# chanzuckerberg/saber

Measured on AMD Instinct MI355X. Metric: EM slices/sec (1024^2, Hiera-L), higher is better.
Workload: dtype bf16; 1 GPU; 1024x1024 uint16 EM slice -> prep.prepare -> SAM2 AMG (Hiera-L, cfgAMG defaults: npoints=32, crop_n_layers=2 -> 21 crops, 3072 grid prompts + 9216 m2m refinements, multimask) -> dedup/sort -> uint16 label plane; BASELINE configs[1]; weights=seeded synthetic Hiera-L (no checkpoint offline), slices_per_rank=22, engine_handles_per_gpu=2, parallelism=single GPU

## Files before the change

include/saber_amd_kernels.h:

```cpp
#ifndef SABER_AMD_KERNELS_H
#define SABER_AMD_KERNELS_H
#include <stdint.h>
#ifdef __cplusplus
extern "C" {
#endif

const char* saber_k_last_error(void);
int saber_k_init(int device_id);

int saber_k_gemm(const uint16_t* A, const uint16_t* W, const float* bias, const float* res, float* out_f32, uint16_t* out_bf16,
                 int M, int N, int K, int act, int act_last, int pool4, int res_shift, int res_mod, void* stream);

int saber_k_gemm_ld(const uint16_t* A, int lda, const uint16_t* W, int ldw, int w_kpad, const float* bias, const float* res, float* out_f32,
                    uint16_t* out_bf16, int M, int N, int K, int act, void* stream);

int saber_k_gemm_rowln(const uint16_t* A, int lda, const uint16_t* W, int ldw, const float* bias, const float* res, float* out_f32,
                       uint16_t* out_bf16, const float* ln_gamma, const float* ln_beta, float ln_eps, uint16_t* ln_out, int M, int N, int K,
                       void* stream);

int saber_k_mlp_rowln(const uint16_t* A, int lda, const uint16_t* W1, int ldw1, const float* b1, const uint16_t* W2, int ldw2, const float* b2,
                      const float* res, float* out_f32, uint16_t* out_bf16, const float* ln_gamma, const float* ln_beta, float ln_eps,
                      uint16_t* ln_out, int M, int C, void* stream);

int saber_k_layernorm(const float* x, const float* gamma, const float* beta, float eps, float* out_f32, uint16_t* out_bf16,
                      int rows, int C, int act, void* stream);

int saber_k_hiera_attention(const uint16_t* qkv, uint16_t* out, int n_windows, int nk, int heads, int q_pool, void* stream);
int saber_k_hiera_attention_ex(const uint16_t* qkv, uint16_t* out, int n_windows, int nk, int heads, int head_dim, int q_pool,
                               const uint8_t* key_mask, void* stream);

int saber_k_dec_attention(const float* q, const float* k, const float* v, uint16_t* out, int B, int nq, int nk, int heads, int hd,
                          int k_shared, void* stream);

int saber_k_prepare(const void* img, int dtype, int H, int W, float* out, float* ws_dev, uint32_t* minmax_dev, void* stream);

int saber_k_mask_post(const float* lowres, int n, int crop_x0, int crop_y0, int crop_w, int crop_h, int H, int W, float thr,
                      float offset, uint32_t* bits, int32_t* stats, void* stream);
// ... 82 lines not shown
```

saber_amd/_lib.py:

```python
import ctypes as C
import os
import subprocess

_HERE = os.path.dirname(os.path.abspath(__file__))
LIB_PATH = os.path.join(_HERE, "libsaber_amd.so")
CSRC = os.path.join(_HERE, "csrc")


class SaberAmdError(RuntimeError):
    pass


class SaberRangeError(SaberAmdError):
    """SABER_ERR_RANGE: the engine's overflow sentinel found NaN / inf in the 16-bit arithmetic (include/saber_amd.h:
    saber_engine_check_finite) - with fp16 operands, an activation beyond 65 504.  The call's results are invalid."""


SABER_OK, SABER_ERR_INVALID, SABER_ERR_STATE, SABER_ERR_HIP, SABER_ERR_CAPACITY, SABER_ERR_RANGE = 0, -1, -2, -3, -4, -5


def build(verbose: bool = False) -> str:
    r = subprocess.run(["make", "-C", CSRC, "-j8"], capture_output=True, text=True)
    if r.returncode != 0:
        raise SaberAmdError("building libsaber_amd.so failed:\n" + r.stdout[-4000:] + r.stderr[-4000:])
# ... 72 lines not shown
    "saber_classifier_set_weight": (_i, [_vp, C.c_char_p, _vp, _i64p, _i]),
    "saber_classifier_finalize": (_i, [_vp]),
    "saber_classifier_predict": (_i, [_vp, _vp, _i, _i, _vp, _i, _i, _vp, _vp]),
    "saber_classifier_head": (_i, [_vp, _vp, _i, _vp, _vp]),
    "saber_classifier_get_crops": (_i, [_vp, _i, _vp, _vp, _vp]),
    "saber_profile_begin": (_i, [_vp]),
    "saber_profile_end": (_i, [_vp, C.POINTER(ProfileClass), _i]),
    "saber_encoder_flops": (C.c_double, [_vp]),
    "saber_decoder_flops_per_prompt": (C.c_double, []),
    "saber_k_last_error": (C.c_char_p, []),
    "saber_k_init": (_i, [_i]),
    "saber_k_gemm": (_i, [_vp, _vp, _vp, _vp, _vp, _vp, _i, _i, _i, _i, _i, _i, _i, _i, _vp]),
    "saber_k_gemm_ld": (_i, [_vp, _i, _vp, _i, _i, _vp, _vp, _vp, _vp, _i, _i, _i, _i, _vp]),
    "saber_k_gemm_rowln": (_i, [_vp, _i, _vp, _i, _vp, _vp, _vp, _vp, _vp, _vp, _f, _vp, _i, _i, _i, _vp]),
    "saber_k_mlp_rowln": (_i, [_vp, _i, _vp, _i, _vp, _vp, _i, _vp, _vp, _vp, _vp, _vp, _vp, _f, _vp, _i, _i, _vp]),
    "saber_k_layernorm": (_i, [_vp, _vp, _vp, _f, _vp, _vp, _i, _i, _i, _vp]),
    "saber_k_hiera_attention": (_i, [_vp, _vp, _i, _i, _i, _i, _vp]),
    "saber_k_hiera_attention_ex": (_i, [_vp, _vp, _i, _i, _i, _i, _i, _vp, _vp]),
    "saber_k_dec_attention": (_i, [_vp, _vp, _vp, _vp, _i, _i, _i, _i, _i, _i, _vp]),
    "saber_k_prepare": (_i, [_vp, _i, _i, _i, _vp, _vp, _vp, _vp]),
    "saber_k_mask_post": (_i, [_vp, _i, _i, _i, _i, _i, _i, _i, _f, _f, _vp, _vp, _vp]),
    "saber_k_perm_index": (_i, [_i, _i, _i]),
    "saber_k_set_operand_type": (_i, [_i]),
    "saber_k_stream_create_cu_range": (_i, [_i, _i, C.POINTER(_vp)]),
    "saber_k_stream_destroy": (_i, [_vp]),
    "saber_k_host_f32_to_f16": (None, [_vp, _vp, C.c_int64]),
    "saber_k_dec_i2t": (_i, [_vp, C.c_int64, _vp, _vp, _vp, _f, _vp, _vp, _vp, _vp, _vp, _f, _vp, _i, _vp]),
    "saber_k_dec_i2t16": (_i, [_vp, C.c_int64, _vp, _vp, _vp, _f, _vp, _vp, _vp, _vp, _vp, _f, _vp, _i, _i, _vp]),
    "saber_k_dec_t2i": (_i, [_vp, C.c_int64, _vp, _vp, _vp, _f, _vp, _vp, _i, _i, _vp, _vp, _vp, _vp]),
    "saber_k_dec_upscale": (_i, [_vp, _vp, _vp, _vp, _vp, _vp, _vp, _vp, _vp, _i, _i, _vp, _vp, _i, _vp, _vp, _i, _vp, _vp]),
# ... 65 lines not shown
```

saber_amd/csrc/capi_kernels.hip:

```cpp
#include <cmath>
#include <cstring>
#include <string>
#include <vector>

#include "../../include/saber_amd_kernels.h"
#include "common.h"
#include "kernels.h"
#include "engine.h"
#include "exact.h"

#include <atomic>

static thread_local std::string g_kerr;
static int kfail(const char* m) { g_kerr = m ? m : "unknown"; return -1; }
static int kcheck(const char* m) {
    if (m) return kfail(m);
    hipError_t st = hipGetLastError();
    if (st != hipSuccess) return kfail(hipGetErrorString(st));
    return 0;
}

extern "C" const char* saber_k_last_error(void) { return g_kerr.c_str(); }

extern "C" int saber_k_init(int device_id) {
    if (hipSetDevice(device_id) != hipSuccess) return kfail("hipSetDevice failed");
    const char* m = gemm_init_device();
    if (!m) m = gemm_rowln_init_device();
    if (!m) m = gemm_mlp_rowln_init_device();
    if (!m) m = hiera_attention_init_device();
    if (!m) m = image_ops_init_device();
    if (!m) m = decoder_fused_init_device();
    if (!m) m = decoder_t16_init_device();
    if (!m) m = amg_device_init();
    (void)hipGetLastError();
    if (m) return kfail(m);
    return 0;
}

extern "C" int saber_k_gemm(const uint16_t* A, const uint16_t* W, const float* bias, const float* res, float* out_f32,
                            uint16_t* out_bf16, int M, int N, int K, int act, int act_last, int pool4, int res_shift, int res_mod,
                            void* stream) {
    GemmParams p;
    p.A = A; p.lda = K; p.W = W; p.ldw = K; p.bias = bias; p.res = res; p.ldres = N; p.Cf = out_f32; p.ldcf = N; p.Cb = out_bf16; p.ldcb = N;
// ... 44 lines not shown
                                 int M, int C, void* stream) {
    if (!gemm_mlp_rowln_width(C)) return kfail("mlp_rowln: width not built (C must be 144)");
    static thread_local bf16_t* scratch = nullptr;
    static thread_local size_t scratch_elems = 0;
    const size_t need = gemm_mlp_rowln_packed_elems(C);
    if (need > scratch_elems) {
        if (scratch) { (void)hipDeviceSynchronize(); (void)hipFree(scratch); scratch = nullptr; scratch_elems = 0; }
        if (hipMalloc(reinterpret_cast<void**>(&scratch), need * sizeof(bf16_t)) != hipSuccess) return kfail("mlp_rowln: scratch allocation failed");
        scratch_elems = need;
    }
    if (const char* m = launch_pack_mlp_chunks(W1, ldw1, W2, ldw2, C, scratch, (hipStream_t)stream)) return kfail(m);
    GemmParams p;
    p.A = A; p.lda = lda; p.bias1 = b1; p.bias = b2; p.res = res; p.ldres = C; p.Cf = out_f32; p.ldcf = C; p.Cb = out_bf16; p.ldcb = C;
    p.M = M; p.N = C; p.K = C; p.ln_gamma = ln_gamma; p.ln_beta = ln_beta; p.ln_eps = ln_eps; p.ln_out = ln_out; p.ldln = C; p.Wpk = scratch;
    return kcheck(launch_gemm_mlp_rowln(p, (hipStream_t)stream));
}

extern "C" int saber_k_layernorm(const float* x, const float* gamma, const float* beta, float eps, float* out_f32, uint16_t* out_bf16,
                                 int rows, int C, int act, void* stream) {
    LayerNormParams p;
    p.x = x; p.ldx = C; p.gamma = gamma; p.beta = beta; p.eps = eps; p.out_f = out_f32; p.out_bf = out_bf16; p.ldo = C; p.rows = rows; p.C = C; p.act = act;
    return kcheck(launch_layernorm(p, (hipStream_t)stream));
}

extern "C" int saber_k_hiera_attention(const uint16_t* qkv, uint16_t* out, int n_windows, int nk, int heads, int q_pool, void* stream) {
    return kcheck(launch_hiera_attention(qkv, out, n_windows, nk, heads, 72, q_pool, nullptr, (hipStream_t)stream));
}

extern "C" int saber_k_hiera_attention_ex(const uint16_t* qkv, uint16_t* out, int n_windows, int nk, int heads, int head_dim, int q_pool,
                                          const uint8_t* key_mask, void* stream) {
// ... 273 lines not shown
```

saber_amd/csrc/engine.h:

```cpp
#pragma once
#include <hip/hip_runtime.h>
#include <functional>
#include <map>
#include <set>
#include <string>
#include <vector>

#include "../../include/saber_amd.h"
#include "kernels.h"

struct BlockSpec { int din, dout, heads, window, q_stride; };

struct HostTensor { std::vector<int64_t> shape; std::vector<float> data; };

struct LinW { const bf16_t* w = nullptr; const float* b = nullptr; int out = 0, in = 0, ldw = 0; const bf16_t* wpk = nullptr; int wpk_n = 0; const float* wf = nullptr;
              const uint8_t* w8 = nullptr; const uint8_t* sw8 = nullptr; int kp8 = 0, sw_rows = 0; };
struct LnW { const float* g = nullptr; const float* b = nullptr; };

struct BlockW { LnW n1, n2; LinW qkv, proj, fc1, fc2, sc; const bf16_t* mlp_pk = nullptr; };

struct AttnW { LinW q, k, v, o; const bf16_t* pe_proj = nullptr; const bf16_t* img_wT = nullptr; };
struct DecLayerW { AttnW self_attn, t2i, i2t; LnW n1, n2, n3, n4; LinW mlp1, mlp2; };

enum { PC_GEMM = 0, PC_HIERA_ATTN, PC_LAYERNORM, PC_DEC_ATTN, PC_ELEMENTWISE, PC_IMAGE, PC_MASK_POST, PC_DEC_T2I, PC_DEC_I2T, PC_DEC_UPSCALE, PC_GEMM_MX, PC_N };
struct ProfRec { int cls; double flops; double bytes; hipEvent_t a, b; };

struct saber_engine {
    int device = 0;
    std::string trunk;
    int max_images = 1, max_prompts = 64;
    std::string err;
    bool finalized = false;
    int weight_format = 0;
    int precision = 0;
// ... 173 lines not shown
```

saber_amd/csrc/engine.hip:

```cpp
#include "engine.h"

#include <algorithm>
#include <cmath>
#include <cstring>
#include <functional>
#include <utility>

#include "common.h"

static thread_local std::string g_create_err;

int eng_fail(saber_engine* e, int code, const std::string& msg) {
    if (e) e->err = msg; else g_create_err = msg;
    return code;
}

int eng_alloc_bytes(saber_engine* e, void** p, size_t bytes) {
    *p = nullptr;
    if (bytes == 0) bytes = 16;
    hipError_t st = hipMalloc(p, bytes);
    if (st != hipSuccess) return eng_fail(e, SABER_ERR_HIP, std::string("hipMalloc(") + std::to_string(bytes) + "): " + hipGetErrorString(st));
    e->allocs.push_back(*p);
    return SABER_OK;
}
// ... 162 lines not shown
    int ndev = 0;
    if (hipGetDeviceCount(&ndev) != hipSuccess || ndev <= 0) return eng_fail(nullptr, SABER_ERR_HIP, "no HIP device visible: the MI355X engine cannot run");
    if (device_id < 0 || device_id >= ndev) return eng_fail(nullptr, SABER_ERR_INVALID, "device_id out of range");
    if (hipSetDevice(device_id) != hipSuccess) return eng_fail(nullptr, SABER_ERR_HIP, "hipSetDevice failed");
    saber_engine* e = new saber_engine();
    e->device = device_id;
    e->trunk = t;
    e->max_images = max_images;
    e->max_prompts = max_prompts;
    if (const char* g = getenv("SABER_AMD_GRAPHS")) e->graphs_on = atoi(g) != 0;
    if (const char* m = hiera_spec(e, *spec)) { delete e; return eng_fail(nullptr, SABER_ERR_INVALID, m); }
    {
        const char* m = gemm_init_device();
            if (!m) m = gemm_rowln_init_device();
            if (!m) m = gemm_mlp_rowln_init_device();
        if (!m) m = amg_device_init();
        if (!m) m = hiera_attention_init_device();
        if (!m) m = image_ops_init_device();
        if (!m) m = decoder_fused_init_device();
        if (!m) m = decoder_tokens_init_device();
        if (!m) m = decoder_t16_init_device();
        (void)hipGetLastError();
        if (m) { delete e; return eng_fail(nullptr, SABER_ERR_HIP, std::string("kernel attribute setup: ") + m); }
    }
    *out = e;
    return SABER_OK;
}

extern "C" void saber_engine_destroy(saber_engine* e) {
    if (!e) return;
// ... 316 lines not shown
            }
        }
        if (!e->padded && (bs.dout == 144 || bs.dout == 288 || bs.dout == 576)) {
            for (LinW* l : {&w.proj, &w.fc2}) {
                bf16_t* d = nullptr;
                TRY(eng_alloc(e, &d, gemm_rowln_packed_elems(l->out, l->in)));
                if (const char* m = launch_pack_w_kstep(l->w, l->ldw, l->out, l->in, d, nullptr)) return eng_fail(e, SABER_ERR_INVALID, m);
                l->wpk = d;
            }
        }
        if (!e->padded && gemm_mlp_rowln_width(bs.dout) && i + 1 < e->blocks.size() && w.fc1.w && w.fc2.w && !w.fc1.w8 && !w.fc2.w8) {
            bf16_t* d = nullptr;
            TRY(eng_alloc(e, &d, gemm_mlp_rowln_packed_elems(bs.dout)));
            if (const char* m = launch_pack_mlp_chunks(w.fc1.w, w.fc1.ldw, w.fc2.w, w.fc2.ldw, bs.dout, d, nullptr)) return eng_fail(e, SABER_ERR_INVALID, m);
            w.mlp_pk = d;
        }
    }
    {
        const std::string nk = "image_encoder.neck.convs.";
        const int dims[4] = {C0 * 8, C0 * 4, C0 * 2, C0};
        const HostTensor *nw[4], *nb[4];
        for (int i = 0; i < 4; ++i) {
            nw[i] = F.get(nk + std::to_string(i) + ".conv.weight", {256, dims[i], 1, 1});
            nb[i] = F.get(nk + std::to_string(i) + ".conv.bias", {256});
        }
        const HostTensor* nm = F.get("no_mem_embed", {1, 1, 256});
        const HostTensor* s0w = F.get("sam_mask_decoder.conv_s0.weight", {32, 256, 1, 1});
        const HostTensor* s0b = F.get("sam_mask_decoder.conv_s0.bias", {32});
        const HostTensor* s1w = F.get("sam_mask_decoder.conv_s1.weight", {64, 256, 1, 1});
        const HostTensor* s1b = F.get("sam_mask_decoder.conv_s1.bias", {64});
// ... 361 lines not shown
    ENG_KP(e, PC_IMAGE, 0.0, 0.0, launch_resize_normalize(img_dev, H, W, channels, e->crops_dev, n, e->pix, 1024, s));
    ENG_KP(e, PC_IMAGE, 0.0, 0.0, launch_patch_embed(e->pix, e->pe_wt, e->pe_bias, e->pos_table, e->xa, n, e->embed_dim, 1024, s));
    if (e->precision == SABER_PRECISION_EXACT) {
        TRY(exact_encode_blocks(e, n, slot0, s));
        for (int i = 0; i < n; ++i) { e->slot_valid[slot0 + i] = 1; e->slot_shared_valid[slot0 + i] = 0; e->slot_embb_valid[slot0 + i] = 0; }
        return SABER_OK;
    }
    float* x = e->xa;
    float* xalt = e->xb;
    int tokens = 65536;
    int stage = 0;
    static const bool no_rowln = getenv("SABER_AMD_NO_ROWLN") != nullptr;
    const bool fuse = !e->padded && !no_rowln;
    static const bool no_mlpfuse = getenv("SABER_AMD_NO_MLPFUSE") != nullptr;
    const bool mlpfuse = fuse && !no_mlpfuse && !(g_saber_debug_flags & 262144);
    const size_t nblocks = e->blocks.size();
    ENG_KP(e, PC_LAYERNORM, 0.0, 0.0, ln_run(x, e->bw[0].n1, 1e-6f, n * tokens, e->blocks[0].din, nullptr, e->xn, ACT_NONE, s, nullptr, nullptr, 0, e->valid[0], tokens));
    const int snake = (g_saber_debug_flags & 512) ? 0 : 1;
    uint8_t* const xn8 = reinterpret_cast<uint8_t*>(e->xn);
    uint8_t* const hid8 = reinterpret_cast<uint8_t*>(e->hid);
    for (size_t i = 0; i < nblocks; ++i) {
        const BlockSpec& bs = e->blocks[i];
        const BlockW& w = e->bw[i];
        const int N = n * tokens;
        float* xres = x;
        int Nq = N;
        if (bs.din != bs.dout) {
            GemmParams g = mk_gemm(e->xn, bs.din, N, w.sc);
            g.Cf = xalt; g.ldcf = bs.dout; g.pool4 = 1;
            ENG_KP(e, PC_GEMM, 2.0 * g.M * (double)g.N * g.K * g.batch, gemm_bytes(g), launch_gemm(g, s));
            xres = xalt;
            Nq = N / 4;
        }
        if (w.qkv.w8) {
            GemmMxParams g = mk_gemm_mx(e, xn8, e->xn8_s, N, w.qkv);
            g.Cb = e->qkv; g.ldcb = 3 * bs.dout;
            ENG_KP(e, PC_GEMM_MX, 2.0 * g.M * (double)g.N * w.qkv.in, (double)g.M * (g.Kp + 2.0 * g.N), launch_gemm_mx(g, s));
        } else {
            GemmParams g = mk_gemm(e->xn, bs.din, N, w.qkv);
            g.Cb = e->qkv; g.ldcb = 3 * bs.dout;
            g.rev = snake;
            ENG_KP(e, PC_GEMM, 2.0 * g.M * (double)g.N * g.K * g.batch, gemm_bytes(g), launch_gemm(g, s));
        }
        const int nk = bs.window > 0 ? bs.window * bs.window : tokens;
        const uint8_t* kmask = (bs.window == 0 && e->valid[stage]) ? e->kmask2 : nullptr;
        ENG_KP(e, PC_HIERA_ATTN, 4.0 * e->head_dim * (double)N * (bs.q_stride > 1 ? nk / 4 : nk) * bs.heads, 0.0,
               launch_hiera_attention(e->qkv, e->att, N / nk, nk, bs.heads, e->head_dim, bs.q_stride > 1, kmask, s));
        {
            GemmParams g = mk_gemm(e->att, bs.dout, Nq, w.proj);
            g.Cf = xres; g.ldcf = bs.dout; g.res = xres; g.ldres = bs.dout;
            g.ln_gamma = w.n2.g; g.ln_beta = w.n2.b; g.ln_eps = 1e-6f; g.ln_out = e->xn; g.ldln = bs.dout;
            g.rev = snake;
            if (w.fc1.w8) {
                g.ln_gamma = nullptr; g.ln_beta = nullptr; g.ln_out = nullptr;
                ENG_KP(e, PC_GEMM, 2.0 * g.M * (double)g.N * g.K * g.batch, gemm_bytes(g), launch_gemm(g, s));
                ENG_KP(e, PC_LAYERNORM, 0.0, 0.0, launch_ln_mx(xres, bs.dout, w.n2.g, w.n2.b, 1e-6f, bs.dout, xn8, mx_kp(bs.dout), mx_kp(bs.dout), e->xn8_s, e->mx_rows, Nq, s));
            } else if (fuse && gemm_rowln_supported(g)) {
                ENG_KP(e, PC_GEMM, 2.0 * g.M * (double)g.N * g.K * g.batch, gemm_bytes(g, true), launch_gemm_rowln(g, s));
            } else {
                ENG_KP(e, PC_GEMM, 2.0 * g.M * (double)g.N * g.K * g.batch, gemm_bytes(g), launch_gemm(g, s));
                ENG_KP(e, PC_LAYERNORM, 0.0, 0.0, ln_run(xres, w.n2, 1e-6f, Nq, bs.dout, nullptr, e->xn, ACT_NONE, s));
            }
        }
        if (bs.din != bs.dout) { std::swap(x, xalt); tokens /= 4; ++stage; }
        const bool has_next = i + 1 < nblocks;
        if (mlpfuse && has_next && w.mlp_pk) {
            GemmParams g = mk_gemm(e->xn, bs.dout, Nq, w.fc2);
            g.K = bs.dout; g.W = nullptr; g.ldw = 0; g.w_kpad = 0; g.Wpk = w.mlp_pk; g.bias1 = w.fc1.b;
            g.Cf = x; g.ldcf = bs.dout; g.res = x; g.ldres = bs.dout;
            g.rev = 0;
            if ((int)i == e->stage_ends[stage]) { g.Cb = e->sb[stage]; g.ldcb = bs.dout; }
            g.ln_gamma = e->bw[i + 1].n1.g; g.ln_beta = e->bw[i + 1].n1.b; g.ln_eps = 1e-6f; g.ln_out = e->xn; g.ldln = bs.dout;
            const double M = g.M, C = bs.dout;
            ENG_KP(e, PC_GEMM, 2.0 * 2.0 * M * C * 4.0 * C, M * C * (2 + 4 + 4 + 2 + (g.Cb ? 2 : 0)) + 2.0 * 8.0 * C * C, launch_gemm_mlp_rowln(g, s));
            continue;
        }
// ... 591 lines not shown
```

saber_amd/csrc/kernels.h:

```cpp
#pragma once
#include <hip/hip_runtime.h>
#include <stdint.h>
#include <stddef.h>

extern int g_saber_debug_flags;
extern unsigned long long* g_saber_stamp_buf;
int saber_cu_count();
extern thread_local int g_saber_op_f16;
inline bool saber_op_is_f16() { return g_saber_op_f16 != 0; }

typedef uint16_t bf16_t;

enum { ACT_NONE = 0, ACT_GELU = 1, ACT_RELU = 2, ACT_SIGMOID = 3 };

struct GemmParams {
    const bf16_t* A = nullptr; int64_t lda = 0; int64_t strideA = 0;
    const bf16_t* W = nullptr; int64_t ldw = 0; int64_t strideW = 0;
    const float* bias = nullptr; int64_t strideBias = 0;
    const float* res = nullptr; int64_t ldres = 0; int64_t strideRes = 0;
    float* Cf = nullptr; int64_t ldcf = 0; int64_t strideCf = 0;
    bf16_t* Cb = nullptr; int64_t ldcb = 0; int64_t strideCb = 0;
    int M = 0, N = 0, K = 0;
    int act = ACT_NONE;
    int act_last = 0;
// ... 114 lines not shown


namespace op_bf16 {
#include "kernels_op.h"
}
namespace op_f16 {
#include "kernels_op.h"
}
#ifndef SABER_OP_NS
#define SABER_OP_FWD(fn)                                                                                                  \
    template <class... A> inline auto fn(A&&... a) {                                                                      \
        return saber_op_is_f16() ? op_f16::fn(static_cast<A&&>(a)...) : op_bf16::fn(static_cast<A&&>(a)...);              \
    }
#define SABER_OP_INIT(fn)                                                                                                 \
    inline const char* fn() { const char* m = op_bf16::fn(); return m ? m : op_f16::fn(); }
SABER_OP_INIT(gemm_init_device) SABER_OP_INIT(gemm_rowln_init_device) SABER_OP_INIT(gemm_mlp_rowln_init_device) SABER_OP_INIT(hiera_attention_init_device)
SABER_OP_INIT(decoder_fused_init_device) SABER_OP_INIT(decoder_tokens_init_device) SABER_OP_INIT(decoder_t16_init_device)
SABER_OP_FWD(launch_gemm) SABER_OP_FWD(gemm_rowln_supported) SABER_OP_FWD(launch_gemm_rowln) SABER_OP_FWD(gemm_rowln_packed_elems) SABER_OP_FWD(launch_pack_w_kstep)
SABER_OP_FWD(gemm_mlp_rowln_width) SABER_OP_FWD(gemm_mlp_rowln_packed_elems) SABER_OP_FWD(launch_pack_mlp_chunks) SABER_OP_FWD(launch_gemm_mlp_rowln)
SABER_OP_FWD(launch_layernorm) SABER_OP_FWD(launch_gather_rows) SABER_OP_FWD(launch_add_to_bf16) SABER_OP_FWD(launch_hiera_attention)
SABER_OP_FWD(launch_prompt_tokens) SABER_OP_FWD(launch_prompt_tokens_multi) SABER_OP_FWD(launch_mask_embed_src) SABER_OP_FWD(launch_mask_hidden) SABER_OP_FWD(launch_embb_tiles)
SABER_OP_FWD(launch_dec_attention) SABER_OP_FWD(launch_mask_pick) SABER_OP_FWD(launch_iou_live_flags) SABER_OP_FWD(launch_mask_select)
SABER_OP_FWD(launch_dec_fold) SABER_OP_FWD(launch_dec_t2i) SABER_OP_FWD(launch_dec_i2t) SABER_OP_FWD(launch_dec_i2t_t2i) SABER_OP_FWD(launch_dec_upscale) SABER_OP_FWD(launch_dec_tokens)
SABER_OP_FWD(launch_prompt_tokens16) SABER_OP_FWD(launch_dec_tokens16) SABER_OP_FWD(launch_dec_i2t16)
SABER_OP_FWD(launch_mask_post) SABER_OP_FWD(launch_gather_masks) SABER_OP_FWD(launch_label_plane) SABER_OP_FWD(launch_pair_intersections) SABER_OP_FWD(launch_unpermute_nchw)
SABER_OP_FWD(launch_rope) SABER_OP_FWD(launch_softmax_rows) SABER_OP_FWD(launch_conv3x3s2) SABER_OP_FWD(launch_unpack_masks) SABER_OP_FWD(launch_paint_nearest)
SABER_OP_FWD(launch_conv3x3s2_t) SABER_OP_FWD(launch_dwconv7_t) SABER_OP_FWD(launch_dwconv7) SABER_OP_FWD(launch_conv4x4s4) SABER_OP_FWD(launch_resize_plane)
SABER_OP_FWD(launch_flash256) SABER_OP_FWD(launch_gauss_mirror) SABER_OP_FWD(launch_axpy) SABER_OP_FWD(launch_bf16_to_f32)
#undef SABER_OP_FWD
#undef SABER_OP_INIT
#endif
```

saber_amd/csrc/kernels_op.h:

```cpp
const char* launch_gemm(const GemmParams& p, hipStream_t stream);
const char* gemm_init_device();
bool gemm_rowln_supported(const GemmParams& p);
const char* launch_gemm_rowln(const GemmParams& p, hipStream_t stream);
const char* gemm_rowln_init_device();
size_t gemm_rowln_packed_elems(int N, int K);
const char* launch_pack_w_kstep(const bf16_t* W, int ldw, int N, int K, bf16_t* out, hipStream_t s);
bool gemm_mlp_rowln_width(int C);
size_t gemm_mlp_rowln_packed_elems(int C);
const char* launch_pack_mlp_chunks(const bf16_t* W1, int ldw1, const bf16_t* W2, int ldw2, int C, bf16_t* out, hipStream_t s);
const char* launch_gemm_mlp_rowln(const GemmParams& p, hipStream_t stream);
const char* gemm_mlp_rowln_init_device();
const char* launch_layernorm(const LayerNormParams& p, hipStream_t s);
const char* launch_gather_rows(const float* in, int64_t in_rows, float* out, int64_t out_rows, const int* idx, int C, int n_images, hipStream_t s);
const char* launch_add_to_bf16(const float* x, const float* y, int ymod, bf16_t* out_bf, float* out_f, int64_t rows, int C,
                               hipStream_t s);
const char* launch_hiera_attention(const bf16_t* qkv, bf16_t* out, int n_windows, int nk, int heads, int hd, int q_pool,
                                   const uint8_t* kmask, hipStream_t s);
const char* hiera_attention_init_device();
const char* launch_prompt_tokens(const float* pts, const int* labels, int P, PromptWeights w, float* tokens, hipStream_t s);
const char* launch_prompt_tokens_multi(const float* pts, const int* labels, int P, int K, PromptWeights w, float* tokens, hipStream_t s);
const char* launch_mask_embed_src(const float* mask_in, int P, const float* image_embed, XMap emb_map, const float* pos, MaskEmbedWeights w,
                                  float* src_f, bf16_t* src_bf, bf16_t* srcpos_bf, float clamp_abs, hipStream_t s, int raw4_q0 = -1);
const char* launch_mask_hidden(const float* mask_in, int P, MaskEmbedWeights w, bf16_t* h2, float clamp_abs, hipStream_t s, int raw4_q0 = -1);
const char* launch_embb_tiles(const float* emb, const float* b3, float* out, hipStream_t s);
const char* launch_dec_attention(const float* q, const float* k, const float* v, bf16_t* out, int B, int nq, int nk, int heads,
                                 int hd, int64_t q_bs, int64_t k_bs, int64_t v_bs, int64_t o_bs, hipStream_t s);
// ... 45 lines not shown
```

Measured before the change: 7.490 slices/s.

## Fuse stage-0 Hiera QKV, windowed attention, projection and LayerNorm into one kernel

Adds a single kernel for stage-0 Hiera blocks (C=144, 2 heads, 8x8 windows). Per 256-row tile it computes the QKV projection, windowed softmax attention and output projection, then applies residual plus LayerNorm, keeping Q in registers and K/V in LDS. Weights are pre-packed into MFMA tile order and double-buffered through LDS. This removes the global round trips for the qkv and attention tensors and two kernel launches per block, at the cost of a narrowly specialised, register- and LDS-heavy kernel with its own packing path.

```diff
diff --git a/include/saber_amd_kernels.h b/include/saber_amd_kernels.h
--- a/include/saber_amd_kernels.h
+++ b/include/saber_amd_kernels.h
@@ -21,6 +21,10 @@
 int saber_k_mlp_rowln(const uint16_t* A, int lda, const uint16_t* W1, int ldw1, const float* b1, const uint16_t* W2, int ldw2, const float* b2,
                       const float* res, float* out_f32, uint16_t* out_bf16, const float* ln_gamma, const float* ln_beta, float ln_eps,
                       uint16_t* ln_out, int M, int C, void* stream);
+
+int saber_k_attn_rowln(const uint16_t* A, int lda, const uint16_t* Wqkv, int ldwqkv, const float* bqkv, const uint16_t* Wp, int ldwp, const float* bp,
+                       const float* res, float* out_f32, uint16_t* out_bf16, const float* ln_gamma, const float* ln_beta, float ln_eps,
+                       uint16_t* ln_out, int M, int C, int heads, void* stream);
 
 int saber_k_layernorm(const float* x, const float* gamma, const float* beta, float eps, float* out_f32, uint16_t* out_bf16,
                       int rows, int C, int act, void* stream);
diff --git a/saber_amd/_lib.py b/saber_amd/_lib.py
--- a/saber_amd/_lib.py
+++ b/saber_amd/_lib.py
@@ -110,6 +110,7 @@
     "saber_k_gemm_ld": (_i, [_vp, _i, _vp, _i, _i, _vp, _vp, _vp, _vp, _i, _i, _i, _i, _vp]),
     "saber_k_gemm_rowln": (_i, [_vp, _i, _vp, _i, _vp, _vp, _vp, _vp, _vp, _vp, _f, _vp, _i, _i, _i, _vp]),
     "saber_k_mlp_rowln": (_i, [_vp, _i, _vp, _i, _vp, _vp, _i, _vp, _vp, _vp, _vp, _vp, _vp, _f, _vp, _i, _i, _vp]),
+    "saber_k_attn_rowln": (_i, [_vp, _i, _vp, _i, _vp, _vp, _i, _vp, _vp, _vp, _vp, _vp, _vp, _f, _vp, _i, _i, _i, _vp]),
     "saber_k_layernorm": (_i, [_vp, _vp, _vp, _f, _vp, _vp, _i, _i, _i, _vp]),
     "saber_k_hiera_attention": (_i, [_vp, _vp, _i, _i, _i, _i, _vp]),
     "saber_k_hiera_attention_ex": (_i, [_vp, _vp, _i, _i, _i, _i, _i, _vp, _vp]),
diff --git a/saber_amd/csrc/attn_rowln.hip b/saber_amd/csrc/attn_rowln.hip
--- /dev/null
+++ b/saber_amd/csrc/attn_rowln.hip
@@ -0,0 +1,327 @@
+#include "common.h"
+#include "kernels.h"
+#include "rowln_epilogue.h"
+
+typedef s16x4 __attribute__((address_space(3))) * lds_s16x4_ptr_a;
+
+template <int C> struct AttnRowLnCfg {
+    static_assert(C == 144, "built for the stage-0 width: 2 heads of 72");
+    static constexpr int R = 256, HD = 72, NK = (C + 31) / 32, NT = C / 16;
+    static constexpr int TPC = 3;
+    static constexpr int QKV_TILES = 36, TILES = QKV_TILES + NT, NCH = TILES / TPC;
+    static constexpr int TILE_B = NK * 1024;
+    static constexpr int UNITS = TPC * TILE_B / 16, NU = (UNITS + 511) / 512;
+    static constexpr int BUF = NU * 512 * 16;
+    static constexpr int VSTRIDE = 224;
+    static constexpr int K_WIN = 4 * 3 * 1024, V_WIN = 64 * VSTRIDE;
+    static constexpr int K_OFF = 0, V_OFF = K_OFF + 4 * K_WIN, W_OFF = V_OFF + 4 * V_WIN, B_OFF = W_OFF + 2 * BUF;
+    static constexpr int SCR_OFF = K_OFF;
+    static constexpr int LDS = B_OFF + QKV_TILES * 16 * 4;
+    static constexpr size_t W_ELEMS = (size_t)TILES * NK * 512;
+    static constexpr size_t PK_ELEMS = W_ELEMS + (size_t)QKV_TILES * 16 * 2;
+    static constexpr float SCALE = 0.11785113019775793f * 1.4426950408889634f;
+    static_assert(8 * RL_SCR <= 4 * K_WIN, "epilogue scratch must fit into the K images");
+    static_assert(TILES % TPC == 0 && (QKV_TILES / 2) % TPC == 0, "chunks must not straddle a head");
+    static_assert(LDS <= 160 * 1024, "LDS budget");
+};
+
+template <int C>
+__global__ __launch_bounds__(512) void gemm_rowln_attn_kernel(GemmParams p) {
+    using CF = AttnRowLnCfg<C>;
+    constexpr int R = CF::R, NK = CF::NK, NT = CF::NT, NCH = CF::NCH, NU = CF::NU, VS = CF::VSTRIDE;
+    static_assert(NT == 9, "rowln_epilogue: 9 column tiles per wave");
+    extern __shared__ __attribute__((aligned(16))) char smem[];
+    const int tid = threadIdx.x, lane = tid & 63;
+    const int wave = __builtin_amdgcn_readfirstlane(tid >> 6);
+    const int fi = lane & 15, fg = lane >> 4;
+    const int win = wave >> 1, half = wave & 1;
+    const int tiles = (p.M + R - 1) / R;
+    int tl = blockIdx.x;
+    if (tl >= tiles) return;
+    auto tile_of = [&](int l) { return p.rev ? tiles - 1 - l : l; };
+
+    float* bs = reinterpret_cast<float*>(smem + CF::B_OFF);
+    for (int i = tid; i < CF::QKV_TILES * 16; i += 512) bs[i] = p.bias1[i];
+
+    const u32x4* __restrict__ wsrc = reinterpret_cast<const u32x4*>(p.Wpk);
+    u32x4 st[NU];
+    auto stage_load = [&](int ch) {
+#pragma unroll
+        for (int q = 0; q < NU; ++q) st[q] = wsrc[(int64_t)ch * CF::UNITS + min(tid + 512 * q, CF::UNITS - 1)];
+    };
+    auto stage_write = [&](int buf) {
+#pragma unroll
+        for (int q = 0; q < NU; ++q) *reinterpret_cast<u32x4*>(smem + CF::W_OFF + buf * CF::BUF + (tid + 512 * q) * 16) = st[q];
+    };
+    op16x8 xn[2][NK];
+    auto load_xn = [&](int tile) {
+        const int rows = min(R, p.M - tile * R);
+        const __amdgpu_buffer_rsrc_t arsrc = __builtin_amdgcn_make_buffer_rsrc((void*)(p.A + (int64_t)tile * R * p.lda), 0, (int)((uint32_t)rows * (uint32_t)p.lda * 2u), 0x00020000);
+        const uint32_t voff = (uint32_t)(((wave * 32 + fi) * (int)p.lda + fg * 8) * 2);
+        const uint32_t istep = (uint32_t)(16 * (int)p.lda * 2);
+#pragma unroll
+        for (int i = 0; i < 2; ++i)
+#pragma unroll
+            for (int ks = 0; ks < NK; ++ks) {
+                u32x4 v = __builtin_amdgcn_raw_buffer_load_b128(arsrc, voff + ks * 64, i * istep, 0);
+                if ((ks + 1) * 32 > C && ks * 32 + fg * 8 >= C) v = (u32x4){0u, 0u, 0u, 0u};
+                xn[i][ks] = __builtin_bit_cast(op16x8, v);
+            }
+    };
+
+    int cur = 0;
+    auto chunk_begin = [&](int next) {
+        stage_load(next);
+        __builtin_amdgcn_sched_barrier(0);
+    };
+    auto chunk_end = [&]() {
+        stage_write(cur ^ 1);
+        __syncthreads();
+        cur ^= 1;
+    };
+    auto xn_tile = [&](int tt, int T, u32x2 (&o)[2]) {
+        const char* wb = smem + CF::W_OFF + cur * CF::BUF + tt * CF::TILE_B + lane * 16;
+        f32x4 t[2] = {(f32x4){0.f, 0.f, 0.f, 0.f}, (f32x4){0.f, 0.f, 0.f, 0.f}};
+#pragma unroll
+        for (int ks = 0; ks < NK; ++ks) {
+            const op16x8 w = *reinterpret_cast<const op16x8*>(wb + ks * 1024);
+#pragma unroll
+            for (int i = 0; i < 2; ++i) t[i] = MFMA_16x16x32(w, xn[i][ks], t[i], 0, 0, 0);
+        }
+        const f32x4 b = *reinterpret_cast<const f32x4*>(bs + T * 16 + fg * 4);
+#pragma unroll
+        for (int i = 0; i < 2; ++i) {
+            o[i][0] = pack_op16(t[i][0] + b[0], t[i][1] + b[1]);
+            o[i][1] = pack_op16(t[i][2] + b[2], t[i][3] + b[3]);
+        }
+    };
+
+    stage_load(0);
+    load_xn(tile_of(tl));
+    stage_write(0);
+    __syncthreads();
+    char* const kimg = smem + CF::K_OFF + win * CF::K_WIN;
+    char* const vimg = smem + CF::V_OFF + win * CF::V_WIN;
+    for (; tl < tiles; tl += gridDim.x) {
+        const int m0 = tile_of(tl) * R;
+        u32x2 att[2][NK][2];
+#pragma unroll
+        for (int h = 0; h < 2; ++h) {
+            const int ch0 = h * 6, T0 = h * 18;
+            u32x2 qh[2][6];
+#pragma unroll
+            for (int c = 0; c < 2; ++c) {
+                chunk_begin(ch0 + c + 1);
+#pragma unroll
+                for (int tt = 0; tt < 3; ++tt) {
+                    u32x2 o[2];
+                    xn_tile(tt, T0 + c * 3 + tt, o);
+                    qh[0][c * 3 + tt] = o[0]; qh[1][c * 3 + tt] = o[1];
+                }
+                chunk_end();
+            }
+#pragma unroll 1
+            for (int c = 0; c < 2; ++c) {
+                chunk_begin(ch0 + 2 + c + 1);
+#pragma unroll
+                for (int tt = 0; tt < 3; ++tt) {
+                    const int t6 = c * 3 + tt;
+                    u32x2 o[2];
+                    xn_tile(tt, T0 + 6 + t6, o);
+#pragma unroll
+                    for (int i = 0; i < 2; ++i)
+                        *reinterpret_cast<u32x2*>(kimg + ((half * 2 + i) * 3 + (t6 >> 1)) * 1024 + lane * 16 + (t6 & 1) * 8) = o[i];
+                }
+                chunk_end();
+            }
+#pragma unroll 1
+            for (int c = 0; c < 2; ++c) {
+                const int nx = ch0 + 4 + c + 1;
+                chunk_begin(nx);
+#pragma unroll
+                for (int tt = 0; tt < 3; ++tt) {
+                    const int t6 = c * 3 + tt;
+                    u32x2 o[2];
+                    xn_tile(tt, T0 + 12 + t6, o);
+#pragma unroll
+                    for (int i = 0; i < 2; ++i)
+                        *reinterpret_cast<u32x2*>(vimg + (half * 32 + i * 16 + fi) * VS + (16 * t6 + 4 * fg) * 2) = o[i];
+                }
+                chunk_end();
+            }
+            f32x4 s[2][4];
+#pragma unroll
+            for (int kt = 0; kt < 4; ++kt) {
+                op16x8 kf[3];
+#pragma unroll
+                for (int c = 0; c < 3; ++c) kf[c] = *reinterpret_cast<const op16x8*>(kimg + (kt * 3 + c) * 1024 + lane * 16);
+#pragma unroll
+                for (int i = 0; i < 2; ++i) {
+                    s[i][kt] = (f32x4){0.f, 0.f, 0.f, 0.f};
+#pragma unroll
+                    for (int c = 0; c < 3; ++c) {
+                        const u32x4 qu = {qh[i][2 * c][0], qh[i][2 * c][1], qh[i][2 * c + 1][0], qh[i][2 * c + 1][1]};
+                        s[i][kt] = MFMA_16x16x32(kf[c], __builtin_bit_cast(op16x8, qu), s[i][kt], 0, 0, 0);
+                    }
+                }
+            }
+            const float sc = CF::SCALE;
+            float inv[2];
+            op16x8 pf[2][2];
+#pragma unroll
+            for (int i = 0; i < 2; ++i) {
+                float mx = -3.0e38f;
+#pragma unroll
+                for (int kt = 0; kt < 4; ++kt)
+#pragma unroll
+                    for (int r = 0; r < 4; ++r) mx = fmaxf(mx, s[i][kt][r]);
+                mx = xor32_max(xor16_max(mx));
+                const float nmx = -mx * sc;
+                float sum = 0.f;
+#pragma unroll
+                for (int kt = 0; kt < 4; ++kt)
+#pragma unroll
+                    for (int r = 0; r < 4; ++r) {
+                        const float e = __builtin_amdgcn_exp2f(fmaf(s[i][kt][r], sc, nmx));
+                        s[i][kt][r] = e;
+                        sum += e;
+                    }
+                sum = xor32_sum(xor16_sum(sum));
+                inv[i] = __builtin_amdgcn_rcpf(sum);
+#pragma unroll
+                for (int ks = 0; ks < 2; ++ks) {
+                    const u32x4 pu = {pack_op16(s[i][2 * ks][0], s[i][2 * ks][1]), pack_op16(s[i][2 * ks][2], s[i][2 * ks][3]),
+                                      pack_op16(s[i][2 * ks + 1][0], s[i][2 * ks + 1][1]), pack_op16(s[i][2 * ks + 1][2], s[i][2 * ks + 1][3])};
+                    pf[i][ks] = __builtin_bit_cast(op16x8, pu);
+                }
+            }
+#pragma unroll
+            for (int T = 0; T < 6; ++T) {
+                f32x4 o[2] = {(f32x4){0.f, 0.f, 0.f, 0.f}, (f32x4){0.f, 0.f, 0.f, 0.f}};
+#pragma unroll
+                for (int ks = 0; ks < 2; ++ks) {
+                    const char* base = vimg + (32 * ks + 4 * fg + (fi >> 2)) * VS + (16 * T + 4 * (fi & 3)) * 2;
+                    const s16x4 lo = __builtin_amdgcn_ds_read_tr16_b64_v4i16((lds_s16x4_ptr_a)(base));
+                    const s16x4 hi = __builtin_amdgcn_ds_read_tr16_b64_v4i16((lds_s16x4_ptr_a)(base + 16 * VS));
+                    const op16x8 vf = __builtin_shufflevector(__builtin_bit_cast(op16x4, lo), __builtin_bit_cast(op16x4, hi), 0, 1, 2, 3, 4, 5, 6, 7);
+#pragma unroll
+                    for (int i = 0; i < 2; ++i) o[i] = MFMA_16x16x32(vf, pf[i][ks], o[i], 0, 0, 0);
+                }
+                const int ksp = 2 * h + (T >> 1), j = T & 1;
+#pragma unroll
+                for (int i = 0; i < 2; ++i) {
+                    u32x2 a;
+                    a[0] = pack_op16(o[i][0] * inv[i], o[i][1] * inv[i]);
+                    a[1] = pack_op16(o[i][2] * inv[i], o[i][3] * inv[i]);
+                    if (h == 1 && ksp == 2) {
+                        a[0] = fg == 0 ? att[i][ksp][j][0] : a[0];
+                        a[1] = fg == 0 ? att[i][ksp][j][1] : a[1];
+                    }
+                    att[i][ksp][j] = a;
+                }
+            }
+        }
+        f32x4 acc[2][9];
+#pragma unroll
+        for (int i = 0; i < 2; ++i)
+#pragma unroll
+            for (int j = 0; j < 9; ++j) acc[i][j] = (f32x4){0.f, 0.f, 0.f, 0.f};
+        op16x8 af[2][NK];
+#pragma unroll
+        for (int i = 0; i < 2; ++i)
+#pragma unroll
+            for (int ks = 0; ks < NK; ++ks) {
+                const u32x4 au = {att[i][ks][0][0], att[i][ks][0][1], att[i][ks][1][0], att[i][ks][1][1]};
+                af[i][ks] = __builtin_bit_cast(op16x8, au);
+            }
+#pragma unroll
+        for (int c = 0; c < 3; ++c) {
+            chunk_begin(c == 2 ? 0 : 12 + c + 1);
+#pragma unroll
+            for (int tt = 0; tt < 3; ++tt) {
+                const char* wb = smem + CF::W_OFF + cur * CF::BUF + tt * CF::TILE_B + lane * 16;
+#pragma unroll
+                for (int ks = 0; ks < NK; ++ks) {
+                    const op16x8 w = *reinterpret_cast<const op16x8*>(wb + ks * 1024);
+#pragma unroll
+                    for (int i = 0; i < 2; ++i) acc[i][c * 3 + tt] = MFMA_16x16x32(w, af[i][ks], acc[i][c * 3 + tt], 0, 0, 0);
+                }
+            }
+            chunk_end();
+        }
+        rowln_epilogue<2, 1, R>(p, acc, m0, wave, 0, wave, lane, static_cast<float*>(nullptr), smem + CF::SCR_OFF, [&] {
+            load_xn(tile_of(tl + (int)gridDim.x < tiles ? tl + (int)gridDim.x : tl));
+        });
+    }
+}
+
+__device__ __forceinline__ int attn_src_row(int T, int fi) {
+    const int h = T / 18, kind = (T % 18) / 6, t6 = T % 6, s = t6 >> 1, j = t6 & 1, g = fi >> 2, r = fi & 3;
+    if (kind < 2) {
+        const int hd = 32 * s + 8 * g + 4 * j + r;
+        return hd < 72 ? kind * 144 + h * 72 + hd : -1;
+    }
+    const int d = 32 * (2 * h + s) + 8 * g + 4 * j + r - 72 * h;
+    return d >= 0 && d < 72 ? 288 + h * 72 + d : -1;
+}
+__global__ __launch_bounds__(256) void pack_attn_tiles_kernel(const bf16_t* __restrict__ Wqkv, int ldq, const float* __restrict__ bqkv, const bf16_t* __restrict__ Wp, int ldp,
+                                                              bf16_t* __restrict__ out) {
+    using CF = AttnRowLnCfg<144>;
+    const int total = CF::TILES * CF::NK * 64;
+    float* bout = reinterpret_cast<float*>(out + CF::W_ELEMS);
+    for (int idx = blockIdx.x * 256 + threadIdx.x; idx < total; idx += gridDim.x * 256) {
+        const int l = idx & 63, f = idx >> 6, T = f / CF::NK, ks = f % CF::NK;
+        const int fi = l & 15, fg = l >> 4, k = ks * 32 + fg * 8;
+        uint4 v = make_uint4(0, 0, 0, 0);
+        if (k < 144) {
+            if (T < CF::QKV_TILES) {
+                const int row = attn_src_row(T, fi);
+                if (row >= 0) v = *reinterpret_cast<const uint4*>(Wqkv + (int64_t)row * ldq + k);
+            } else {
+                v = *reinterpret_cast<const uint4*>(Wp + (int64_t)((T - CF::QKV_TILES) * 16 + fi) * ldp + k);
+            }
+        }
+        *reinterpret_cast<uint4*>(out + (int64_t)idx * 8) = v;
+        if (idx < CF::QKV_TILES * 16) {
+            const int row = attn_src_row(idx >> 4, idx & 15);
+            bout[idx] = (row >= 0 && bqkv) ? bqkv[row] : 0.f;
+        }
+    }
+}
+
+bool gemm_attn_rowln_shape(int C, int heads) { return C == 144 && heads == 2; }
+size_t gemm_attn_rowln_packed_elems() { return AttnRowLnCfg<144>::PK_ELEMS; }
+const char* launch_pack_attn_tiles(const bf16_t* Wqkv, int ldwqkv, const float* bqkv, const bf16_t* Wp, int ldwp, int C, int heads, bf16_t* out, hipStream_t s) {
+    if (!gemm_attn_rowln_shape(C, heads)) return "pack_attn_tiles: shape not built (C = 144, 2 heads)";
+    if ((ldwqkv & 7) || ldwqkv < C || (ldwp & 7) || ldwp < C) return "pack_attn_tiles: ldwqkv / ldwp must be multiples of 8 and cover the rows";
+    if (!Wqkv || !Wp || !out || ((uintptr_t)Wqkv & 15) || ((uintptr_t)Wp & 15) || ((uintptr_t)out & 15) || ((uintptr_t)bqkv & 3)) return "pack_attn_tiles: operand alignment";
+    const int total = AttnRowLnCfg<144>::TILES * AttnRowLnCfg<144>::NK * 64;
+    hipLaunchKernelGGL(pack_attn_tiles_kernel, dim3((unsigned)((total + 255) / 256)), dim3(256), 0, s, Wqkv, ldwqkv, bqkv, Wp, ldwp, out);
+    return nullptr;
+}
+
+const char* gemm_attn_rowln_init_device() {
+    const hipError_t st = hipFuncSetAttribute(reinterpret_cast<const void*>(gemm_rowln_attn_kernel<144>), hipFuncAttributeMaxDynamicSharedMemorySize, AttnRowLnCfg<144>::LDS);
+    return st == hipSuccess ? nullptr : hipGetErrorString(st);
+}
+
+const char* launch_gemm_attn_rowln(const GemmParams& p_in, hipStream_t stream) {
+    GemmParams p = p_in;
+    p.dbg = g_saber_debug_flags;
+    if (!gemm_attn_rowln_shape(p.N, 2) || p.K != p.N || !p.Wpk || !p.Cf || !p.ln_out || !p.ln_gamma || !p.ln_beta || p.batch > 1 || p.pool4 || p.act != ACT_NONE ||
+        p.res_shift || p.res_mod)
+        return "gemm_attn_rowln: unsupported problem (C must be 144; packed weights, fp32 + LayerNorm outputs required)";
+    if (p.M <= 0) return "gemm_attn_rowln: empty problem";
+    if (p.M % 64) return "gemm_attn_rowln: M must be a multiple of the 64-row window";
+    if ((p.lda & 7) || p.lda < p.N) return "gemm_attn_rowln: lda must be a multiple of 8 and cover the row";
+    if (((uintptr_t)p.A & 15) || ((uintptr_t)p.Wpk & 15) || ((uintptr_t)p.Cf & 15) || (p.ldcf & 3) || ((uintptr_t)p.ln_out & 7) || (p.ldln & 3) ||
+        (p.res && (((uintptr_t)p.res & 15) || (p.ldres & 3))) || (p.bias && ((uintptr_t)p.bias & 15)) ||
+        (p.Cb && (((uintptr_t)p.Cb & 7) || (p.ldcb & 3))) || ((uintptr_t)p.ln_gamma & 15) || ((uintptr_t)p.ln_beta & 15))
+        return "gemm_attn_rowln: operand alignment";
+    if ((int64_t)p.M * p.lda >= ((int64_t)1 << 40)) return "gemm_attn_rowln: problem too large";
+    p.bias1 = reinterpret_cast<const float*>(p.Wpk + AttnRowLnCfg<144>::W_ELEMS);
+    const int n_cu = saber_cu_count();
+    const int tiles = (p.M + AttnRowLnCfg<144>::R - 1) / AttnRowLnCfg<144>::R;
+    hipLaunchKernelGGL((gemm_rowln_attn_kernel<144>), dim3(tiles < n_cu ? tiles : n_cu), dim3(512), AttnRowLnCfg<144>::LDS, stream, p);
+    return nullptr;
+}
diff --git a/saber_amd/csrc/capi_kernels.hip b/saber_amd/csrc/capi_kernels.hip
--- a/saber_amd/csrc/capi_kernels.hip
+++ b/saber_amd/csrc/capi_kernels.hip
@@ -27,6 +27,7 @@
     const char* m = gemm_init_device();
     if (!m) m = gemm_rowln_init_device();
     if (!m) m = gemm_mlp_rowln_init_device();
+    if (!m) m = gemm_attn_rowln_init_device();
     if (!m) m = hiera_attention_init_device();
     if (!m) m = image_ops_init_device();
     if (!m) m = decoder_fused_init_device();
@@ -101,6 +102,27 @@
     p.A = A; p.lda = lda; p.bias1 = b1; p.bias = b2; p.res = res; p.ldres = C; p.Cf = out_f32; p.ldcf = C; p.Cb = out_bf16; p.ldcb = C;
     p.M = M; p.N = C; p.K = C; p.ln_gamma = ln_gamma; p.ln_beta = ln_beta; p.ln_eps = ln_eps; p.ln_out = ln_out; p.ldln = C; p.Wpk = scratch;
     return kcheck(launch_gemm_mlp_rowln(p, (hipStream_t)stream));
+}
+
+extern "C" int saber_k_attn_rowln(const uint16_t* A, int lda, const uint16_t* Wqkv, int ldwqkv, const float* bqkv, const uint16_t* Wp, int ldwp, const float* bp,
+                                  const float* res, float* out_f32, uint16_t* out_bf16, const float* ln_gamma, const float* ln_beta, float ln_eps, uint16_t* ln_out,
+                                  int M, int C, int heads, void* stream) {
+    if (C != 144) return kfail("attn_rowln: width not built (C must be 144)");
+    if (heads != 2) return kfail("attn_rowln: heads must be 2 (head_dim 72)");
+    if (M <= 0 || (M % 64)) return kfail("attn_rowln: M must be a positive multiple of the 64-row window");
+    static thread_local bf16_t* scratch_dev[64] = {nullptr};
+    int dev = 0;
+    if (hipGetDevice(&dev) != hipSuccess || dev < 0 || dev >= 64) return kfail("attn_rowln: no current device");
+    bf16_t*& scratch = scratch_dev[dev];
+    if (!scratch && hipMalloc(reinterpret_cast<void**>(&scratch), gemm_attn_rowln_packed_elems() * sizeof(bf16_t)) != hipSuccess) {
+        scratch = nullptr;
+        return kfail("attn_rowln: scratch allocation failed");
+    }
+    if (const char* m = launch_pack_attn_tiles(Wqkv, ldwqkv, bqkv, Wp, ldwp, C, heads, scratch, (hipStream_t)stream)) return kfail(m);
+    GemmParams p;
+    p.A = A; p.lda = lda; p.bias = bp; p.res = res; p.ldres = C; p.Cf = out_f32; p.ldcf = C; p.Cb = out_bf16; p.ldcb = C;
+    p.M = M; p.N = C; p.K = C; p.ln_gamma = ln_gamma; p.ln_beta = ln_beta; p.ln_eps = ln_eps; p.ln_out = ln_out; p.ldln = C; p.Wpk = scratch;
+    return kcheck(launch_gemm_attn_rowln(p, (hipStream_t)stream));
 }
 
 extern "C" int saber_k_layernorm(const float* x, const float* gamma, const float* beta, float eps, float* out_f32, uint16_t* out_bf16,
diff --git a/saber_amd/csrc/engine.h b/saber_amd/csrc/engine.h
--- a/saber_amd/csrc/engine.h
+++ b/saber_amd/csrc/engine.h
@@ -17,7 +17,7 @@
               const uint8_t* w8 = nullptr; const uint8_t* sw8 = nullptr; int kp8 = 0, sw_rows = 0; };
 struct LnW { const float* g = nullptr; const float* b = nullptr; };
 
-struct BlockW { LnW n1, n2; LinW qkv, proj, fc1, fc2, sc; const bf16_t* mlp_pk = nullptr; };
+struct BlockW { LnW n1, n2; LinW qkv, proj, fc1, fc2, sc; const bf16_t* mlp_pk = nullptr; const bf16_t* attn_pk = nullptr; };
 
 struct AttnW { LinW q, k, v, o; const bf16_t* pe_proj = nullptr; const bf16_t* img_wT = nullptr; };
 struct DecLayerW { AttnW self_attn, t2i, i2t; LnW n1, n2, n3, n4; LinW mlp1, mlp2; };
diff --git a/saber_amd/csrc/engine.hip b/saber_amd/csrc/engine.hip
--- a/saber_amd/csrc/engine.hip
+++ b/saber_amd/csrc/engine.hip
@@ -200,6 +200,7 @@
         const char* m = gemm_init_device();
             if (!m) m = gemm_rowln_init_device();
             if (!m) m = gemm_mlp_rowln_init_device();
+            if (!m) m = gemm_attn_rowln_init_device();
         if (!m) m = amg_device_init();
         if (!m) m = hiera_attention_init_device();
         if (!m) m = image_ops_init_device();
@@ -546,6 +547,13 @@
             TRY(eng_alloc(e, &d, gemm_mlp_rowln_packed_elems(bs.dout)));
             if (const char* m = launch_pack_mlp_chunks(w.fc1.w, w.fc1.ldw, w.fc2.w, w.fc2.ldw, bs.dout, d, nullptr)) return eng_fail(e, SABER_ERR_INVALID, m);
             w.mlp_pk = d;
+        }
+        if (!e->padded && bs.din == bs.dout && gemm_attn_rowln_shape(bs.dout, bs.heads) && e->head_dim == 72 && bs.window == 8 && bs.q_stride == 1 && w.qkv.w && w.proj.w &&
+            !w.qkv.w8 && !w.proj.w8) {
+            bf16_t* d = nullptr;
+            TRY(eng_alloc(e, &d, gemm_attn_rowln_packed_elems()));
+            if (const char* m = launch_pack_attn_tiles(w.qkv.w, w.qkv.ldw, w.qkv.b, w.proj.w, w.proj.ldw, bs.dout, bs.heads, d, nullptr)) return eng_fail(e, SABER_ERR_INVALID, m);
+            w.attn_pk = d;
         }
     }
     {
@@ -937,6 +945,8 @@
     const bool fuse = !e->padded && !no_rowln;
     static const bool no_mlpfuse = getenv("SABER_AMD_NO_MLPFUSE") != nullptr;
     const bool mlpfuse = fuse && !no_mlpfuse && !(g_saber_debug_flags & 262144);
+    static const bool no_attnfuse = getenv("SABER_AMD_NO_ATTNFUSE") != nullptr;
+    const bool attnfuse = fuse && !no_attnfuse && !(g_saber_debug_flags & 524288);
     const size_t nblocks = e->blocks.size();
     ENG_KP(e, PC_LAYERNORM, 0.0, 0.0, ln_run(x, e->bw[0].n1, 1e-6f, n * tokens, e->blocks[0].din, nullptr, e->xn, ACT_NONE, s, nullptr, nullptr, 0, e->valid[0], tokens));
     const int snake = (g_saber_debug_flags & 512) ? 0 : 1;
@@ -955,34 +965,44 @@
             xres = xalt;
             Nq = N / 4;
         }
-        if (w.qkv.w8) {
-            GemmMxParams g = mk_gemm_mx(e, xn8, e->xn8_s, N, w.qkv);
-            g.Cb = e->qkv; g.ldcb = 3 * bs.dout;
-            ENG_KP(e, PC_GEMM_MX, 2.0 * g.M * (double)g.N * w.qkv.in, (double)g.M * (g.Kp + 2.0 * g.N), launch_gemm_mx(g, s));
-        } else {
-            GemmParams g = mk_gemm(e->xn, bs.din, N, w.qkv);
-            g.Cb = e->qkv; g.ldcb = 3 * bs.dout;
-            g.rev = snake;
-            ENG_KP(e, PC_GEMM, 2.0 * g.M * (double)g.N * g.K * g.batch, gemm_bytes(g), launch_gemm(g, s));
-        }
-        const int nk = bs.window > 0 ? bs.window * bs.window : tokens;
-        const uint8_t* kmask = (bs.window == 0 && e->valid[stage]) ? e->kmask2 : nullptr;
-        ENG_KP(e, PC_HIERA_ATTN, 4.0 * e->head_dim * (double)N * (bs.q_stride > 1 ? nk / 4 : nk) * bs.heads, 0.0,
-               launch_hiera_attention(e->qkv, e->att, N / nk, nk, bs.heads, e->head_dim, bs.q_stride > 1, kmask, s));
-        {
-            GemmParams g = mk_gemm(e->att, bs.dout, Nq, w.proj);
-            g.Cf = xres; g.ldcf = bs.dout; g.res = xres; g.ldres = bs.dout;
+        if (attnfuse && w.attn_pk && bs.din == bs.dout && bs.window == 8 && bs.q_stride == 1) {
+            GemmParams g = mk_gemm(e->xn, bs.dout, N, w.proj);
+            g.W = nullptr; g.ldw = 0; g.w_kpad = 0; g.Wpk = w.attn_pk;
+            g.Cf = x; g.ldcf = bs.dout; g.res = x; g.ldres = bs.dout;
             g.ln_gamma = w.n2.g; g.ln_beta = w.n2.b; g.ln_eps = 1e-6f; g.ln_out = e->xn; g.ldln = bs.dout;
             g.rev = snake;
-            if (w.fc1.w8) {
-                g.ln_gamma = nullptr; g.ln_beta = nullptr; g.ln_out = nullptr;
+            const double M = N, C = bs.dout, nk = 64;
+            ENG_KP(e, PC_GEMM, 2.0 * M * C * 3.0 * C + 4.0 * M * nk * C + 2.0 * M * C * C, M * C * (2 + 4 + 4 + 2) + 2.0 * 4.0 * C * C, launch_gemm_attn_rowln(g, s));
+        } else {
+            if (w.qkv.w8) {
+                GemmMxParams g = mk_gemm_mx(e, xn8, e->xn8_s, N, w.qkv);
+                g.Cb = e->qkv; g.ldcb = 3 * bs.dout;
+                ENG_KP(e, PC_GEMM_MX, 2.0 * g.M * (double)g.N * w.qkv.in, (double)g.M * (g.Kp + 2.0 * g.N), launch_gemm_mx(g, s));
+            } else {
+                GemmParams g = mk_gemm(e->xn, bs.din, N, w.qkv);
+                g.Cb = e->qkv; g.ldcb = 3 * bs.dout;
+                g.rev = snake;
                 ENG_KP(e, PC_GEMM, 2.0 * g.M * (double)g.N * g.K * g.batch, gemm_bytes(g), launch_gemm(g, s));
-                ENG_KP(e, PC_LAYERNORM, 0.0, 0.0, launch_ln_mx(xres, bs.dout, w.n2.g, w.n2.b, 1e-6f, bs.dout, xn8, mx_kp(bs.dout), mx_kp(bs.dout), e->xn8_s, e->mx_rows, Nq, s));
-            } else if (fuse && gemm_rowln_supported(g)) {
-                ENG_KP(e, PC_GEMM, 2.0 * g.M * (double)g.N * g.K * g.batch, gemm_bytes(g, true), launch_gemm_rowln(g, s));
-            } else {
-                ENG_KP(e, PC_GEMM, 2.0 * g.M * (double)g.N * g.K * g.batch, gemm_bytes(g), launch_gemm(g, s));
-                ENG_KP(e, PC_LAYERNORM, 0.0, 0.0, ln_run(xres, w.n2, 1e-6f, Nq, bs.dout, nullptr, e->xn, ACT_NONE, s));
+            }
+            const int nk = bs.window > 0 ? bs.window * bs.window : tokens;
+            const uint8_t* kmask = (bs.window == 0 && e->valid[stage]) ? e->kmask2 : nullptr;
+            ENG_KP(e, PC_HIERA_ATTN, 4.0 * e->head_dim * (double)N * (bs.q_stride > 1 ? nk / 4 : nk) * bs.heads, 0.0,
+                   launch_hiera_attention(e->qkv, e->att, N / nk, nk, bs.heads, e->head_dim, bs.q_stride > 1, kmask, s));
+            {
+                GemmParams g = mk_gemm(e->att, bs.dout, Nq, w.proj);
+                g.Cf = xres; g.ldcf = bs.dout; g.res = xres; g.ldres = bs.dout;
+                g.ln_gamma = w.n2.g; g.ln_beta = w.n2.b; g.ln_eps = 1e-6f; g.ln_out = e->xn; g.ldln = bs.dout;
+                g.rev = snake;
+                if (w.fc1.w8) {
+                    g.ln_gamma = nullptr; g.ln_beta = nullptr; g.ln_out = nullptr;
+                    ENG_KP(e, PC_GEMM, 2.0 * g.M * (double)g.N * g.K * g.batch, gemm_bytes(g), launch_gemm(g, s));
+                    ENG_KP(e, PC_LAYERNORM, 0.0, 0.0, launch_ln_mx(xres, bs.dout, w.n2.g, w.n2.b, 1e-6f, bs.dout, xn8, mx_kp(bs.dout), mx_kp(bs.dout), e->xn8_s, e->mx_rows, Nq, s));
+                } else if (fuse && gemm_rowln_supported(g)) {
+                    ENG_KP(e, PC_GEMM, 2.0 * g.M * (double)g.N * g.K * g.batch, gemm_bytes(g, true), launch_gemm_rowln(g, s));
+                } else {
+                    ENG_KP(e, PC_GEMM, 2.0 * g.M * (double)g.N * g.K * g.batch, gemm_bytes(g), launch_gemm(g, s));
+                    ENG_KP(e, PC_LAYERNORM, 0.0, 0.0, ln_run(xres, w.n2, 1e-6f, Nq, bs.dout, nullptr, e->xn, ACT_NONE, s));
+                }
             }
         }
         if (bs.din != bs.dout) { std::swap(x, xalt); tokens /= 4; ++stage; }
diff --git a/saber_amd/csrc/kernels.h b/saber_amd/csrc/kernels.h
--- a/saber_amd/csrc/kernels.h
+++ b/saber_amd/csrc/kernels.h
@@ -152,10 +152,11 @@
     }
 #define SABER_OP_INIT(fn)                                                                                                 \
     inline const char* fn() { const char* m = op_bf16::fn(); return m ? m : op_f16::fn(); }
-SABER_OP_INIT(gemm_init_device) SABER_OP_INIT(gemm_rowln_init_device) SABER_OP_INIT(gemm_mlp_rowln_init_device) SABER_OP_INIT(hiera_attention_init_device)
+SABER_OP_INIT(gemm_init_device) SABER_OP_INIT(gemm_rowln_init_device) SABER_OP_INIT(gemm_mlp_rowln_init_device) SABER_OP_INIT(gemm_attn_rowln_init_device) SABER_OP_INIT(hiera_attention_init_device)
 SABER_OP_INIT(decoder_fused_init_device) SABER_OP_INIT(decoder_tokens_init_device) SABER_OP_INIT(decoder_t16_init_device)
 SABER_OP_FWD(launch_gemm) SABER_OP_FWD(gemm_rowln_supported) SABER_OP_FWD(launch_gemm_rowln) SABER_OP_FWD(gemm_rowln_packed_elems) SABER_OP_FWD(launch_pack_w_kstep)
 SABER_OP_FWD(gemm_mlp_rowln_width) SABER_OP_FWD(gemm_mlp_rowln_packed_elems) SABER_OP_FWD(launch_pack_mlp_chunks) SABER_OP_FWD(launch_gemm_mlp_rowln)
+SABER_OP_FWD(gemm_attn_rowln_shape) SABER_OP_FWD(gemm_attn_rowln_packed_elems) SABER_OP_FWD(launch_pack_attn_tiles) SABER_OP_FWD(launch_gemm_attn_rowln)
 SABER_OP_FWD(launch_layernorm) SABER_OP_FWD(launch_gather_rows) SABER_OP_FWD(launch_add_to_bf16) SABER_OP_FWD(launch_hiera_attention)
 SABER_OP_FWD(launch_prompt_tokens) SABER_OP_FWD(launch_prompt_tokens_multi) SABER_OP_FWD(launch_mask_embed_src) SABER_OP_FWD(launch_mask_hidden) SABER_OP_FWD(launch_embb_tiles)
 SABER_OP_FWD(launch_dec_attention) SABER_OP_FWD(launch_mask_pick) SABER_OP_FWD(launch_iou_live_flags) SABER_OP_FWD(launch_mask_select)
diff --git a/saber_amd/csrc/kernels_op.h b/saber_amd/csrc/kernels_op.h
--- a/saber_amd/csrc/kernels_op.h
+++ b/saber_amd/csrc/kernels_op.h
@@ -10,6 +10,11 @@
 const char* launch_pack_mlp_chunks(const bf16_t* W1, int ldw1, const bf16_t* W2, int ldw2, int C, bf16_t* out, hipStream_t s);
 const char* launch_gemm_mlp_rowln(const GemmParams& p, hipStream_t stream);
 const char* gemm_mlp_rowln_init_device();
+bool gemm_attn_rowln_shape(int C, int heads);
+size_t gemm_attn_rowln_packed_elems();
+const char* launch_pack_attn_tiles(const bf16_t* Wqkv, int ldwqkv, const float* bqkv, const bf16_t* Wp, int ldwp, int C, int heads, bf16_t* out, hipStream_t s);
+const char* launch_gemm_attn_rowln(const GemmParams& p, hipStream_t stream);
+const char* gemm_attn_rowln_init_device();
 const char* launch_layernorm(const LayerNormParams& p, hipStream_t s);
 const char* launch_gather_rows(const float* in, int64_t in_rows, float* out, int64_t out_rows, const int* idx, int C, int n_images, hipStream_t s);
 const char* launch_add_to_bf16(const float* x, const float* y, int ymod, bf16_t* out_bf, float* out_f, int64_t rows, int C,
```

Measured after the change: 7.539 slices/s, median of 6. No clear change (+0.7%).
